# illini-robomaster/irmv_detection

Measured on AMD Instinct MI355X. Metric: end-to-end FPS (preprocess→NMS→PnP) 640×640 YOLOv8n, 1/2/4/8 MI355X, higher is better.
Workload: dtype f16

## Files before the change

include/irmv_hip.h:

```cpp
#ifndef IRMV_HIP_H
#define IRMV_HIP_H

#include <stddef.h>
#include <stdint.h>

#ifdef __cplusplus
extern "C" {
#endif

#define IRMV_OK 0
#define IRMV_ERR_ARG (-1)
#define IRMV_ERR_HIP (-2)
#define IRMV_ERR_MODEL (-3)

#define IRMV_RESIZE_STRETCH 0
#define IRMV_RESIZE_LETTERBOX 1

#define IRMV_ARMOR_SMALL 0
#define IRMV_ARMOR_LARGE 1

#define IRMV_POINTS_AUTO 0
#define IRMV_POINTS_KEYPOINT_HEAD 1
#define IRMV_POINTS_CLASSICAL 2

// ... 119 lines not shown
int irmv_engine_detect(irmv_engine *e, int slot, irmv_det *out, int cap, int *n);
double irmv_engine_last_detect_ms(const irmv_engine *e);

int irmv_engine_rotated_image(irmv_engine *e, int slot, uint8_t *dst_hwc);

int irmv_engine_extract_armors(irmv_engine *e, int slot, const float *xyxy, int n, irmv_det *out);
int irmv_engine_set_extract_params(irmv_engine *e, int binary_threshold, float light_min_ratio, float light_max_ratio,
                                   float light_max_angle, const double center_distances[4]);
int irmv_engine_point_source(const irmv_engine *e);

int irmv_engine_read_input(irmv_engine *e, int slot, float *chw);
int irmv_engine_read_head(irmv_engine *e, int slot, float *head);
int irmv_engine_write_head(irmv_engine *e, int slot, const float *head);
int irmv_engine_run_post(irmv_engine *e, int first_slot, int count);
int irmv_engine_debug_poke_candidate_counts(irmv_engine *e, int value);
int irmv_engine_read_tap(irmv_engine *e, int slot, const char *name, float *nhwc, int shape[3]);
int irmv_engine_read_raw(irmv_engine *e, int slot, irmv_raw_dets *out);
int irmv_engine_num_anchors(const irmv_engine *e);
int irmv_engine_head_channels(const irmv_engine *e);
int irmv_engine_net_dims(const irmv_engine *e, int *width, int *height);

typedef struct irmv_conv_seg {
    char tensor[32];
    int32_t coff, C, shift;
} irmv_conv_seg;

typedef struct irmv_conv_op {
    int32_t op;
    char layer[32];
    int32_t ks, stride, act, out_f32, cin, cout, cout_pad;
// ... 86 lines not shown
```

irmv_detection_amd/capi.py:

```python
from __future__ import annotations

import ctypes as C
import os

from . import _build

OK, ERR_ARG, ERR_HIP, ERR_MODEL = 0, -1, -2, -3
RESIZE_STRETCH, RESIZE_LETTERBOX = 0, 1
ARMOR_SMALL, ARMOR_LARGE = 0, 1
SUBMIT_H2D = 1
SUBMIT_ASYNC_UPLOAD = 2
POINTS_AUTO, POINTS_KEYPOINT_HEAD, POINTS_CLASSICAL = 0, 1, 2
SRC_HWC8, SRC_BAYER_RGGB8, SRC_BAYER_BGGR8, SRC_BAYER_GRBG8, SRC_BAYER_GBRG8 = 0, 1, 2, 3, 4
BAYER_FORMATS = {"RGGB": SRC_BAYER_RGGB8, "BGGR": SRC_BAYER_BGGR8, "GRBG": SRC_BAYER_GRBG8, "GBRG": SRC_BAYER_GBRG8}
NUM_CLASSES = 14
MAX_DET_CAP = 256
CAND_CAP = 8192


class IrmvError(RuntimeError):
    def __init__(self, code: int, msg: str):
        super().__init__(f"irmv_hip error {code}: {msg}")
        self.code = code

# ... 119 lines not shown
    ("irmv_engine_wait_upload", C.c_int, [_P, C.c_int, C.c_int]),
    ("irmv_engine_set_extract_params", C.c_int, [_P, C.c_int, C.c_float, C.c_float, C.c_float, C.POINTER(C.c_double)]),
    ("irmv_engine_point_source", C.c_int, [_P]),
    ("irmv_engine_results", C.c_int, [_P, C.c_int, C.POINTER(Det), C.c_int, C.POINTER(C.c_int)]),
    ("irmv_engine_detect", C.c_int, [_P, C.c_int, C.POINTER(Det), C.c_int, C.POINTER(C.c_int)]),
    ("irmv_engine_last_detect_ms", C.c_double, [_P]),
    ("irmv_engine_rotated_image", C.c_int, [_P, C.c_int, C.POINTER(C.c_uint8)]),
    ("irmv_engine_extract_armors", C.c_int, [_P, C.c_int, C.POINTER(C.c_float), C.c_int, C.POINTER(Det)]),
    ("irmv_engine_light_trace", C.c_int, [_P, C.c_int, C.POINTER(C.c_float), C.c_int, C.POINTER(LightTrace), C.POINTER(Det)]),
    ("irmv_light_limits", C.c_int, [C.POINTER(C.c_int32)]),
    ("irmv_engine_read_input", C.c_int, [_P, C.c_int, C.POINTER(C.c_float)]),
    ("irmv_engine_read_head", C.c_int, [_P, C.c_int, C.POINTER(C.c_float)]),
    ("irmv_engine_write_head", C.c_int, [_P, C.c_int, C.POINTER(C.c_float)]),
    ("irmv_engine_run_post", C.c_int, [_P, C.c_int, C.c_int]),
    ("irmv_engine_debug_poke_candidate_counts", C.c_int, [_P, C.c_int]),
    ("irmv_engine_read_tap", C.c_int, [_P, C.c_int, C.c_char_p, C.POINTER(C.c_float), C.POINTER(C.c_int)]),
    ("irmv_engine_read_raw", C.c_int, [_P, C.c_int, C.POINTER(RawDets)]),
    ("irmv_engine_num_anchors", C.c_int, [_P]),
    ("irmv_engine_head_channels", C.c_int, [_P]),
    ("irmv_engine_net_dims", C.c_int, [_P, C.POINTER(C.c_int), C.POINTER(C.c_int)]),
    ("irmv_engine_conv_ops", C.c_int, [_P, C.POINTER(ConvOp), C.c_int, C.POINTER(C.c_int)]),
    ("irmv_engine_conv_candidates", C.c_int, [_P, C.c_int, C.c_int, C.POINTER(ConvCand), C.c_int, C.POINTER(C.c_int)]),
    ("irmv_engine_run_conv_candidate", C.c_int, [_P, C.c_int, C.c_int, C.c_int, C.c_int, C.c_int, C.c_uint32]),
    ("irmv_engine_read_tensor", C.c_int, [_P, C.c_char_p, C.c_int, C.c_int, C.c_void_p, C.c_size_t]),
    ("irmv_engine_ops", C.c_int, [_P, C.POINTER(GraphOp), C.c_int, C.POINTER(C.c_int)]),
    ("irmv_engine_run_op", C.c_int, [_P, C.c_int, C.c_int, C.c_int, C.c_uint32]),
    ("irmv_sppf_slab", C.c_int, [C.c_int, C.c_int, C.c_int, C.c_int]),
    ("irmv_engine_profile", C.c_int, [_P, C.c_int, C.c_int, C.POINTER(KernelStat), C.c_int, C.POINTER(C.c_int)]),
    ("irmv_pnp_create", C.c_int, [C.c_int, C.POINTER(C.c_double), C.POINTER(C.c_double), C.POINTER(_P)]),
    ("irmv_pnp_destroy", None, [_P]),
# ... 64 lines not shown
```

irmv_detection_amd/csrc/engine.cpp:

```cpp
#include <hip/hip_runtime.h>

#include <algorithm>
#include <chrono>
#include <cmath>
#include <cstdio>
#include <cstring>
#include <fstream>
#include <map>
#include <mutex>
#include <set>
#include <memory>
#include <string>
#include <vector>

#include "../../include/irmv_hip.h"
#include "irmv_common.hpp"
#include "numa.hpp"

using namespace irmv;

static thread_local std::string g_err;
static int fail(int code, const std::string &msg)
{
    g_err = msg;
// ... 133 lines not shown
    bool fused_away = false;
    int group = -1;
    int bneck = -1;
    int kpt3 = -1;
    int tune_fuse[2] = {-1, -1};
};

enum StepKind { STEP_BATCH, STEP_ONE, STEP_MATERIALIZE, STEP_POST };

struct Launch {
    int op = -1, group = -1;
    bool cfg_one = false;
    bool fused = false;
    unsigned scan = 0;
    bool keys_only = false;
    bool once = false;
    std::string name, layer;
    double flops = 0, bytes = 0, launch_bytes = 0;
};

struct GraphKey {
    int first, count;
    StepKind kind;
    bool upload;
    bool operator<(const GraphKey &o) const { return std::tie(first, count, kind, upload) < std::tie(o.first, o.count, o.kind, o.upload); }
};

struct SlotGroup {
    int first = 0, count = 0;
    hipEvent_t h2d = nullptr, out = nullptr;
// ... 3 lines not shown
};

struct irmv_engine {
    irmv_engine_cfg cfg{};
    int nc = 0, nk = 0, A = 0, no = 0;
    int backbone = 0;
    int num_cus = 256;
    int numa_node = -1;
    bool numa_placed = false;
    struct HeadGroup { std::vector<int> members; int family = 0, nt = 1; ConvCfg cfg{}; char name[48] = {0}; };
    std::vector<HeadGroup> head_groups;
    bool post_keys_only = false;
    bool emit_scan = false;
    bool split_scan = true;
    int *cand_counts = nullptr;
    int lvl_hw[3] = {0, 0, 0}, lvl_base[3] = {0, 0, 0};
    size_t frame_bytes = 0;
    size_t src_bytes = 0;
    hipStream_t stream = nullptr;
    hipStream_t extra_streams[7] = {nullptr, nullptr, nullptr, nullptr, nullptr, nullptr, nullptr};
    int num_streams = 1;
    hipStream_t h2d_stream = nullptr;
    std::map<std::pair<int, int>, SlotGroup> groups;
    std::vector<SlotGroup *> slot_owner;
    bool inline_copies = false;
    bool graph_upload = true;
    uint8_t *src_host = nullptr;
    int sync_launch = 0;
    uint8_t *src_host_dev = nullptr;
    int upload_kernel_blocks = 256;
// ... 813 lines not shown
                if (!(fh && fh[0] == '0') && o1.cout == 64 && o1.cin % 32 == 0 && o1.pair && o1.res_t < 0 && o1.cfg.stride == 1 &&
                    o2.cin == 64 && o2.ksteps == 2 && o2.cfg.ks == 1 && o2.cfg.out_f32 && o2.cfg.act == 0 && (o2.cout_pad == 16 || o2.cout_pad == 64))
                    e->ops[i1].fuse_next = i2;
                if (!(fh && fh[0] == '0') && o1.cfg.cin16 && o1.cout_pad == 16 && !o1.pair && o1.res_t < 0 && o1.cfg.stride == 1 && o1.cfg.act == 1 && o2.w_k16)
                    e->ops[i1].fuse_next = i2;
            }
            if (b == 2 && !e->merge_head0) TRY(fuse_kpt3(e, i));
        }

    TRY(dev_alloc(e, (void **)&e->boxes, (size_t)S * e->A * 16));
    TRY(dev_alloc(e, (void **)&e->keys, (size_t)S * e->A * e->nc * 8));
    { const char *sp = getenv("IRMV_SPLIT_SCAN"); e->split_scan = !(sp && sp[0] == '0'); }
    if (e->split_scan) {
        TRY(dev_alloc(e, (void **)&e->cand_counts, (size_t)S * sizeof(int)));
        HIP_TRY(hipMemset(e->cand_counts, 0, (size_t)S * sizeof(int)));
    }
    TRY(dev_alloc(e, (void **)&e->dets_dev, (size_t)S * c.max_det * sizeof(DevDet)));
    TRY(dev_alloc(e, (void **)&e->fout_dev, (size_t)S * sizeof(DevFrameOut)));
    HIP_TRY(hipMemset(e->dets_dev, 0, (size_t)S * c.max_det * sizeof(DevDet)));
    HIP_TRY(hipMemset(e->fout_dev, 0, (size_t)S * sizeof(DevFrameOut)));
    HIP_TRY(hipHostMalloc((void **)&e->dets_host, (size_t)S * c.max_det * sizeof(DevDet), hipHostMallocMapped | hipHostMallocCoherent));
    HIP_TRY(hipHostMalloc((void **)&e->fout_host, (size_t)S * sizeof(DevFrameOut), hipHostMallocMapped | hipHostMallocCoherent));
    HIP_TRY(hipHostGetDevicePointer((void **)&e->dets_host_dev, e->dets_host, 0));
    HIP_TRY(hipHostGetDevicePointer((void **)&e->fout_host_dev, e->fout_host, 0));
    log_range(e, "pinned dets_host", e->dets_host, (size_t)S * c.max_det * sizeof(DevDet));
    log_range(e, "pinned fout_host", e->fout_host, (size_t)S * sizeof(DevFrameOut));
    memset(e->dets_host, 0, (size_t)S * c.max_det * sizeof(DevDet));
    memset(e->fout_host, 0, (size_t)S * sizeof(DevFrameOut));
    if (e->split_scan) {
        Op op; op.kind = OP_SCAN; op.layer = "scan_decode"; snprintf(op.kname, sizeof op.kname, "scan_decode");
        op.bytes = (double)e->A * 64.0; e->ops.push_back(op);
// ... 536 lines not shown
    for (Op &op : e->ops) {
        if (op.fuse_next < 0) continue;
        const bool k16 = op.cfg.cin16 && !op.cfg.lds && !op.cfg_one.lds && !op.cfg.deep && !op.cfg_one.deep && op.cfg.nt == 1 && op.cfg_one.nt == 1 && e->ops[op.fuse_next].w_k16;
        const bool ok = k16 || (op.cfg.lds && op.cfg.nt == 4 && op.cfg_one.lds && op.cfg_one.nt == 4);
        if (!ok) { op.fuse_next = -1; continue; }
        e->ops[op.fuse_next].fused_away = true;
        e->lazy_tensors.insert(e->tensors[op.out_t].name);
        const size_t l = strlen(op.kname), l1 = strlen(op.kname_one);
        snprintf(op.kname + l, sizeof op.kname - l, "+1x1");
        snprintf(op.kname_one + l1, sizeof op.kname_one - l1, "+1x1");
    }
    int fused = 0;
    for (const Op &op : e->ops) fused += is_cls_final_carrier(op);
    const char *ev = getenv("IRMV_EMIT_SCAN");
    e->emit_scan = e->split_scan && fused == 3 && !(ev && ev[0] == '0');
}

static void scan_args_for(const irmv_engine *e, const Op &op, const PostArgs &pa, ConvArgs &a)
{
    a.scan_keys = pa.keys; a.scan_counts = pa.counts; a.scan_thr = pa.logit_thr; a.scan_nc = pa.nc;
    a.scan_key_cap = pa.key_cap;
    a.scan_abase = e->lvl_base[op.level];
}

static bool launch_head_group(const irmv_engine *e, const irmv_engine::HeadGroup &g, int first, const PostArgs *pa, unsigned scan, hipStream_t s)
{
    ConvArgs a[kMultiMax];
    ConvWeights w[kMultiMax];
    const int n = (int)g.members.size();
    for (int k = 0; k < n; k++) {
        const Op &op = e->ops[g.members[k]];
        fill_conv_args(e, op, first, 1, a[k], true);
        if (scan >> k & 1u) scan_args_for(e, op, *pa, a[k]);
        w[k] = conv_weights(op);
    }
    return g.family == 0 ? launch_conv_lds_multi(g.nt, a, w, n, 1, s) : launch_conv_direct_multi(g.cfg, a, n, s);
}
// ... 81 lines not shown
        if (kpt) { g3.push_back(find_op("model.22.cv4." + si + ".1")); g4.push_back(find_op("model.22.cv4." + si + ".2")); }
    }
    try_group(g1, 0, {1, 2}, "head_s0");
    if (g2_fused) try_group(g2, 0, {4}, "head_s1+1x1");
    if (kpt) {
        const size_t before = e->head_groups.size();
        try_group(g3, 1, {1}, "head_kpt1");
        bool k16 = false;
        for (int i : g4) k16 = k16 || i < 0 || e->ops[i].w_k16 != nullptr;
        if (e->head_groups.size() > before && !k16) try_group(g4, 1, {1}, "head_kpt2");
    }
    HIP_TRY(hipStreamSynchronize(e->stream));
    return IRMV_OK;
}

static void build_step_plans(irmv_engine *e)
{
    for (int k = STEP_BATCH; k <= STEP_POST; k++) {
        const bool one = k == STEP_ONE, mat = k == STEP_MATERIALIZE, post = k == STEP_POST, step = !mat && !post;
        auto emits = [&](const Op &op) { return step && e->emit_scan && is_cls_final_carrier(op); };
        for (int i = 0; i < (int)e->ops.size(); i++) {
            const Op &op = e->ops[i];
            if (post && op.kind != OP_NMS && op.kind != OP_LIGHT && op.kind != OP_SCAN) continue;
            if (op.kind == OP_SCAN && e->emit_scan && !post) continue;
            const bool grouped = one && op.kind == OP_CONV && op.group >= 0;
            if (grouped && e->head_groups[op.group].members[0] != i) continue;
            const bool bneck = one && e->bneck64;
            if (op.kind == OP_BNECK ? !bneck : (op.bneck >= 0 && bneck)) continue;
            if (op.kind == OP_KPT3 ? !step : (op.kpt3 >= 0 && step)) continue;
            if (mat ? !(op.fused_away || op.fuse_next >= 0 || ((op.bneck >= 0 || op.kpt3 >= 0) && op.kind == OP_CONV)) : op.fused_away) continue;
// ... 12 lines not shown
                    l.flops += mo.flops + (mo.fuse_next >= 0 ? e->ops[mo.fuse_next].flops : 0.0);
                    l.bytes += mo.bytes;
                }
            } else {
                l.cfg_one = op.kind == OP_CONV && (one || mat) && stream_share(e, e->cfg.num_slots) > 1;
                l.fused = !mat && op.fuse_next >= 0;
                l.scan = emits(op) ? 1u : 0u;
                l.name = l.cfg_one ? op.kname_one : op.kname;
                const Op *nx = l.fused ? &e->ops[op.fuse_next] : nullptr;
                l.flops = op.flops + (nx ? nx->flops : 0.0);
                l.launch_bytes = op.w_bytes + (nx ? nx->w_bytes : 0.0);
                l.bytes = op.bytes + (nx ? nx->out_bytes - op.out_bytes + nx->w_bytes : 0.0) - l.launch_bytes;
            }
            e->plans[k].push_back(l);
        }
    }
}

struct EvRec { hipEvent_t a = nullptr, b = nullptr; };
constexpr int kProfileRepeat = 4;

static void fill_conv_args(const irmv_engine *e, const Op &op, int first, int count, ConvArgs &a, bool fused)
{
    a = ConvArgs{};
    auto seg = [&](const SegRef &s) {
        ConvSeg cs{nullptr, 0, 0, 0};
        if (s.t < 0 || s.C == 0) return cs;
        const Tensor &t = e->tensors[s.t];
        cs.p = static_cast<const half_t *>(t.slot(first)) + s.coff;
        cs.ld = t.C;
// ... 69 lines not shown
}

static PostArgs post_args(const irmv_engine *e, int first)
{
    PostArgs p = e->post;
    p.head_all = e->head_all;
    p.slots_total = e->cfg.num_slots;
    p.first = first;
    p.boxes = e->boxes + (size_t)first * e->A * 4;
    p.keys = e->keys + (size_t)first * e->A * e->nc;
    p.key_cap = e->A * e->nc;
    p.dets = (e->zero_copy_results ? e->dets_host_dev : e->dets_dev) + (size_t)first * e->cfg.max_det;
    p.fout = (e->zero_copy_results ? e->fout_host_dev : e->fout_dev) + first;
    if (p.dbg) p.dbg += (size_t)first * 16;
    p.counts = e->split_scan ? e->cand_counts + first : nullptr;
    return p;
}

static bool launch_c2f32_op(const irmv_engine *e, const Op &op, int first, int count, hipStream_t s)
{
    C2f32Args a{};
    const Tensor &ct = e->tensors[op.res_t];
    const Tensor &ot = e->tensors[op.out_t];
    if (op.sub[0] >= 0) {
        ConvArgs ca;
        fill_conv_args(e, e->ops[op.sub[0]], first, count, ca, false);
        a.s0 = ca.s0; a.s1 = ca.s1; a.cin1 = ca.Cin;
        a.w_cv1 = e->ops[op.sub[0]].w_packed; a.b_cv1 = e->ops[op.sub[0]].bias;
    } else {
        a.cin1 = 32;
// ... 127 lines not shown
            }
            if (!launch_bneck64(op.mode, ks2, op.shortcut, a, count, s)) return fail(IRMV_ERR_ARG, "no fused bottleneck kernel for " + op.layer);
            break;
        }
        case OP_KPT3: {
            const Op &o0 = e->ops[op.sub[0]], &o1 = e->ops[op.sub[1]], &o2 = e->ops[op.sub[2]];
            const Tensor &xt = e->tensors[o0.s0.t], &ht = e->tensors[o2.out_t];
            Kpt3Args a{};
            a.x = static_cast<const half_t *>(xt.slot(first)) + o0.s0.coff; a.x_ld = xt.C;
            a.H = op.Hin; a.W = op.Win;
            a.tiles_x = (op.Win + kKpt3Tile - 1) / kKpt3Tile; a.tiles_y = (op.Hin + kKpt3Tile - 1) / kKpt3Tile;
            a.w1 = o0.w_lds[0]; a.b1 = o0.bias;
            a.w2 = o1.w_packed; a.b2 = o1.bias;
            a.w3 = o2.w_k16; a.b3 = o2.bias;
            a.out = static_cast<float *>(ht.slot(first)) + o2.out_coff; a.out_ld = ht.C;
            if (!launch_kpt3(a, op.cin, count, s)) return fail(IRMV_ERR_ARG, "no fused keypoint-branch kernel for " + op.layer);
            break;
        }
        case OP_DW: case OP_SHUF: case OP_CONV0: case OP_POOL: launch_graph_op(e, op, first, count, s); break;
        case OP_CONV: {
            const unsigned scan = rep == n - 1 ? l.scan : 0u;
            if (l.group >= 0) {
                if (!launch_head_group(e, e->head_groups[l.group], first, &pa, scan, s)) return fail(IRMV_ERR_ARG, "grouped launch refused: " + l.name);
                break;
            }
            ConvArgs a;
            fill_conv_args(e, op, first, count, a, l.fused);
            if (scan) scan_args_for(e, op, pa, a);
            if (!run_conv(op, l.cfg_one ? op.cfg_one : op.cfg, a, count, s)) return fail(IRMV_ERR_ARG, std::string("no conv kernel for ") + op.kname + " (" + op.layer + ")");
            break;
        }
        case OP_SCAN: launch_scan_decode(pa, count, s); break;
        case OP_NMS: { PostArgs pn = pa; pn.keys_only = l.keys_only ? 1 : 0; launch_nms_pnp(pn, count, s); break; }
        case OP_LIGHT: launch_light_extract(light_args(e, first), e->cfg.max_det, count, s); break;
        }
        HIP_TRY(hipGetLastError());
        if (ev) {
            HIP_TRY(hipEventRecord(r.b, s));
            ev->push_back(r);
        }
    }
    return IRMV_OK;
}
// ... 95 lines not shown
        if (up != st) HIP_TRY(hipStreamWaitEvent(up, o->out, 0));
    }
    if (g->in_flight && g->compute != st) HIP_TRY(hipStreamWaitEvent(st, g->out, 0));
    if (flags & IRMV_SUBMIT_H2D) {
        if (async_up) {
            if (g->in_flight) HIP_TRY(hipStreamWaitEvent(up, g->out, 0));
            TRY(copy_in(e, f, c, up));
            HIP_TRY(hipEventRecord(g->h2d, up));
            HIP_TRY(hipStreamWaitEvent(st, g->h2d, 0));
        } else if (!graph_up) {
            TRY(upload_sync(e, f, c, st));
        }
    }
    if (eager) TRY(enqueue_step(e, kind, f, c, st, 1, nullptr));
    else HIP_TRY(hipGraphLaunch(ge, st));
    TRY(copy_out(e, f, c, st));
    HIP_TRY(hipEventRecord(g->out, st));
    g->in_flight = true;
    g->async_up = async_up;
    g->compute = st;
    return IRMV_OK;
}

extern "C" int irmv_engine_submit(irmv_engine *e, int first, int count, uint32_t flags)
{
    TRY(check_range(e, first, count));
    HIP_TRY(hipSetDevice(e->cfg.device));
    int share = count > 1 ? stream_share(e, count) : count;
    int si = count == 1 ? first % e->num_streams : 0;
    const int full_share = stream_share(e, e->cfg.num_slots);
// ... 7 lines not shown
}

extern "C" int irmv_engine_wait(irmv_engine *e);

extern "C" int irmv_engine_debug_poke_candidate_counts(irmv_engine *e, int value)
{
    if (!e) return fail(IRMV_ERR_ARG, "engine is null");
    if (!e->cand_counts) return fail(IRMV_ERR_ARG, "this engine keeps no candidate counters");
    TRY(irmv_engine_wait(e));
    HIP_TRY(hipSetDevice(e->cfg.device));
    std::vector<int> v((size_t)e->cfg.num_slots, value);
    HIP_TRY(hipMemcpy(e->cand_counts, v.data(), v.size() * sizeof(int), hipMemcpyHostToDevice));
    return IRMV_OK;
}

extern "C" int irmv_engine_run_post(irmv_engine *e, int first, int count)
{
    TRY(check_range(e, first, count));
    HIP_TRY(hipSetDevice(e->cfg.device));
    TRY(irmv_engine_wait(e));
    hipGraphExec_t ge;
    TRY(get_graph(e, STEP_POST, first, count, false, &ge));
    HIP_TRY(hipGraphLaunch(ge, e->stream));
    TRY(copy_out(e, first, count));
    HIP_TRY(hipStreamSynchronize(e->stream));
    return IRMV_OK;
}

extern "C" int irmv_engine_wait(irmv_engine *e)
{
    if (!e) return fail(IRMV_ERR_ARG, "engine is null");
    HIP_TRY(hipSetDevice(e->cfg.device));
    HIP_TRY(hipStreamSynchronize(e->h2d_stream));
    HIP_TRY(hipStreamSynchronize(e->stream));
    for (int i = 1; i < e->num_streams; i++) HIP_TRY(hipStreamSynchronize(e->extra_streams[i - 1]));
// ... 200 lines not shown
        std::vector<uint16_t> h(t.slot_elems);
        HIP_TRY(hipMemcpy(h.data(), t.slot(slot), t.slot_elems * 2, hipMemcpyDeviceToHost));
        const float unscale = t.name == "input" ? 1.0f : kActUnscale;
        for (size_t i = 0; i < t.slot_elems; i++) out[i] = half_bits_to_float(h[i]) * unscale;
    }
    return IRMV_OK;
}

static int materialize_fused(irmv_engine *e, int slot)
{
    if (e->lazy_tensors.empty()) return IRMV_OK;
    HIP_TRY(hipSetDevice(e->cfg.device));
    TRY(irmv_engine_wait(e));
    TRY(enqueue_step(e, STEP_MATERIALIZE, slot, 1, e->stream, 1, nullptr));
    HIP_TRY(hipStreamSynchronize(e->stream));
    return IRMV_OK;
}

extern "C" int irmv_engine_read_input(irmv_engine *e, int slot, float *chw)
{
    TRY(check_range(e, slot, 1));
    TRY(materialize_fused(e, slot));
    std::vector<float> v;
    TRY(read_tensor_f32(e, e->tensors[e->tensor_idx.at("input")], slot, v));
    const size_t n = (size_t)e->cfg.net_size * e->cfg.net_height;
    for (size_t p = 0; p < n; p++)
        for (int c = 0; c < 3; c++) chw[c * n + p] = v[p * 4 + c];
    return IRMV_OK;
}

extern "C" int irmv_engine_read_head(irmv_engine *e, int slot, float *head)
{
    TRY(check_range(e, slot, 1));
    for (int l = 0; l < 3; l++) {
        std::vector<float> v;
        TRY(read_tensor_f32(e, e->tensors[e->head_t[l]], slot, v));
        for (int p = 0; p < e->lvl_hw[l]; p++) {
            float *o = head + (size_t)(e->lvl_base[l] + p) * e->no;
            const float *r = v.data() + (size_t)p * kHeadRec;
            memcpy(o, r, 64 * 4);
            memcpy(o + 64, r + kClsOff, (size_t)e->nc * 4);
            if (e->nk) memcpy(o + 64 + e->nc, r + kKptOff, (size_t)e->nk * 4);
        }
    }
    return IRMV_OK;
}

extern "C" int irmv_engine_write_head(irmv_engine *e, int slot, const float *head)
{
    TRY(check_range(e, slot, 1));
    HIP_TRY(hipSetDevice(e->cfg.device));
    TRY(irmv_engine_wait(e));
    for (int l = 0; l < 3; l++) {
        std::vector<float> v((size_t)e->lvl_hw[l] * kHeadRec, 0.f);
        for (int p = 0; p < e->lvl_hw[l]; p++) {
            const float *o = head + (size_t)(e->lvl_base[l] + p) * e->no;
            float *r = v.data() + (size_t)p * kHeadRec;
            memcpy(r, o, 64 * 4);
            memcpy(r + kClsOff, o + 64, (size_t)e->nc * 4);
            if (e->nk) memcpy(r + kKptOff, o + 64 + e->nc, (size_t)e->nk * 4);
        }
        HIP_TRY(hipMemcpy(e->tensors[e->head_t[l]].slot(slot), v.data(), v.size() * 4, hipMemcpyHostToDevice));
    }
    return IRMV_OK;
}

extern "C" int irmv_engine_read_tap(irmv_engine *e, int slot, const char *name, float *nhwc, int shape[3])
{
    TRY(check_range(e, slot, 1));
    if (!name || !shape) return fail(IRMV_ERR_ARG, "name/shape is null");
    auto it = e->tensor_idx.find(name);
    if (it == e->tensor_idx.end()) return fail(IRMV_ERR_ARG, std::string("no tensor named ") + name);
    const Tensor &t = e->tensors[it->second];
    shape[0] = t.H; shape[1] = t.W; shape[2] = t.C;
    if (!nhwc) return IRMV_OK;
    if (e->lazy_tensors.count(t.name)) TRY(materialize_fused(e, slot));
    std::vector<float> v;
    TRY(read_tensor_f32(e, t, slot, v));
    memcpy(nhwc, v.data(), v.size() * 4);
    return IRMV_OK;
}

extern "C" int irmv_engine_read_tensor(irmv_engine *e, const char *name, int first, int count, void *dst, size_t bytes)
{
    TRY(check_range(e, first, count));
    if (!name) return fail(IRMV_ERR_ARG, "name is null");
    auto it = e->tensor_idx.find(name);
    if (it == e->tensor_idx.end()) return fail(IRMV_ERR_ARG, std::string("no tensor named ") + name);
    const Tensor &t = e->tensors[it->second];
    const size_t need = t.slot_elems * t.esize() * count;
    if (!dst || bytes != need) return fail(IRMV_ERR_ARG, "read_tensor: buffer size does not match the slot range");
    TRY(irmv_engine_wait(e));
    HIP_TRY(hipMemcpy(dst, t.slot(first), need, hipMemcpyDeviceToHost));
    return IRMV_OK;
}

static int conv_op_at(const irmv_engine *e, int op)
{
    if (!e) return fail(IRMV_ERR_ARG, "engine is null");
    if (op < 0 || op >= (int)e->ops.size() || e->ops[op].kind != OP_CONV) return fail(IRMV_ERR_ARG, "not a conv op");
    return IRMV_OK;
}

extern "C" int irmv_engine_conv_ops(irmv_engine *e, irmv_conv_op *ops, int cap, int *n)
{
    if (!e || !n) return fail(IRMV_ERR_ARG, "engine / n is null");
    auto name = [](char *dst, size_t cap_, const std::string &s) { snprintf(dst, cap_, "%s", s.c_str()); };
// ... 224 lines not shown
        if (out->det_anchors) out->det_anchors[i] = d[i].anchor;
        if (out->det_kpts) memcpy(out->det_kpts + 8 * i, d[i].kpts_net, 32);
    }
    return IRMV_OK;
}

extern "C" int irmv_engine_profile(irmv_engine *e, int first, int count, irmv_kernel_stat *stats, int cap, int *n)
{
    TRY(check_range(e, first, count));
    if (!n) return fail(IRMV_ERR_ARG, "n is null");
    HIP_TRY(hipSetDevice(e->cfg.device));
    TRY(irmv_engine_wait(e));
    const StepKind kind = count == 1 ? STEP_ONE : STEP_BATCH;
    std::vector<EvRec> ev;
    TRY(enqueue_step(e, kind, first, count, e->stream, kProfileRepeat, &ev));
    TRY(copy_out(e, first, count));
    HIP_TRY(hipStreamSynchronize(e->stream));
    for (size_t i = 0; i < ev.size(); i++) {
        float ms = 0.f;
        HIP_TRY(hipEventElapsedTime(&ms, ev[i].a, ev[i].b));
        (void)hipEventDestroy(ev[i].a);
        (void)hipEventDestroy(ev[i].b);
        const Launch &l = e->plans[kind][i];
        if ((int)i < cap && stats) {
            irmv_kernel_stat &st = stats[i];
            memset(&st, 0, sizeof st);
            snprintf(st.name, sizeof st.name, "%s", l.name.c_str());
            snprintf(st.layer, sizeof st.layer, "%s", l.layer.c_str());
            st.flops = l.flops * count;
            st.bytes = l.bytes * count + l.launch_bytes;
// ... 78 lines not shown
```

irmv_detection_amd/csrc/irmv_common.hpp:

```cpp
#pragma once

#include <hip/hip_runtime.h>

#include <cstdint>
#include <cstdlib>

namespace irmv {

typedef _Float16 half_t;
typedef _Float16 half8 __attribute__((ext_vector_type(8)));
typedef _Float16 half4 __attribute__((ext_vector_type(4)));
typedef float f32x4 __attribute__((ext_vector_type(4)));

constexpr float kActScale = 1.44269504088896341f;
constexpr float kActUnscale = 0.693147180559945309f;
typedef unsigned int u32x4_t __attribute__((ext_vector_type(4)));
__device__ __forceinline__ float silu_rcp(float y) { return __builtin_amdgcn_rcpf(1.0f + __builtin_amdgcn_exp2f(-y)); }
__device__ __forceinline__ unsigned int silu_pack2(float y0, float y1)
{
    const float r0 = silu_rcp(y0), r1 = silu_rcp(y1);
    unsigned int o;
    asm("v_fma_mixlo_f16 %0, %1, %2, 0" : "=v"(o) : "v"(y0), "v"(r0));
    asm("v_fma_mixhi_f16 %0, %1, %2, 0" : "+v"(o) : "v"(y1), "v"(r1));
    return o;
// ... 180 lines not shown
bool launch_bneck64(int mode, int ks2, bool shortcut, const BneckArgs &a, int batch, hipStream_t s);

constexpr int kKpt3Tile = 10;
struct Kpt3Args {
    const half_t *x;
    int x_ld;
    int H, W, tiles_x, tiles_y;
    const half_t *w1;
    const float *b1;
    const half_t *w2;
    const float *b2;
    const half_t *w3;
    const float *b3;
    float *out;
    int out_ld;
};
bool kpt3_eligible(int cin);
bool launch_kpt3(const Kpt3Args &a, int cin, int batch, hipStream_t s);

struct ConvArgs {
    ConvSeg s0, s1;
    int Hin, Win;
    int Hout, Wout;
    int M;
    int Cin;
    const half_t *w;
    const float *bias;
    void *out;
    int out_ld;
    const half_t *res;
    int res_ld;
    int cout_pad;
    int ksteps;
    int pair;
    const half_t *w2;
    const float *bias2;
    float *out2;
    int out2_ld, n2;
    unsigned long long *scan_keys;
    int *scan_counts;
    float scan_thr;
    int scan_nc, scan_abase, scan_key_cap;
};

constexpr int kMultiMax = 6;
struct LdsMember {
    ConvArgs a;
    const half_t *wl;
    int tiles_x, tiles_y, twc_log2, patch_bytes, batch, tile2d;
    int gx, gy;
};
struct LdsMultiArgs {
    int n;
    int start[kMultiMax + 1];
    LdsMember m[kMultiMax];
};
struct DirectMultiArgs {
// ... 55 lines not shown
    unsigned long long *keys;
    int key_cap;
    DevDet *dets;
    DevFrameOut *fout;
    int net_w, net_h, A, nc, nk;
    float logit_thr, iou_thr;
    int max_det, pre_nms_cap;
    float scale_x, scale_y, off_x, off_y;
    int armor_size;
    const PnpConst *pnp;
    long long *dbg;
    int keys_only;
    int prefilter;
    int classwalk;
    int *counts;
};
void launch_nms_pnp(const PostArgs &a, int batch, hipStream_t s);
constexpr int kScanBlocks = 16;
constexpr size_t kScanLdsMax = 159 * 1024;
void launch_scan_decode(const PostArgs &a, int batch, hipStream_t s);
constexpr int kLightLdsPoints = 256;
constexpr int kLightLdsImage = 40 * 1024;
constexpr int kLightMaxContours = 1024;
constexpr int kLightPointsCap = 4096;

struct LightTraceRec {
    float corners[8];
    float top[2], bottom[2], center[2];
    double length;
    int32_t measured, ok, hull_edges, in_lds;
// ... 40 lines not shown
```

irmv_detection_amd/csrc/k_conv.hip:

```cpp
#include "irmv_common.hpp"

#include <algorithm>
#include <cstdio>
#include <cstring>
#include <iterator>
#include <mutex>
#include <type_traits>

namespace irmv {

template <int MT, int NT>
struct PrefetchDepth { static constexpr int value = (MT * NT >= 8) ? 2 : ((MT * NT >= 4) ? 3 : 4); };
template <int MT, int NT>
struct DeepPrefetchDepth { static constexpr int value = (MT + NT <= 2) ? 12 : ((MT + NT <= 3) ? 10 : 6); };


template <int KS, int STRIDE, int MT, int NT, bool CIN16, int ACT, bool OUT_F32, bool CT = false, bool DEEP = false>
__device__ __forceinline__ void conv_mfma_body(const ConvArgs &a, int wg_x, int wg_y, int grid_x, int grid_y)
{
    constexpr int PAD = KS / 2;
    constexpr int PF = DEEP ? DeepPrefetchDepth<MT, NT>::value : PrefetchDepth<MT, NT>::value;
    static_assert(!CT || (KS == 3 && !CIN16), "chunk-major order is the 3x3 LDS family's");
    const int lane = threadIdx.x & 63, wave = threadIdx.x >> 6;
    const int g = lane >> 4, r = lane & 15;
// ... 818 lines not shown
            for (int mt = 0; mt < MT; mt++) {
                const size_t m = (size_t)im * HWo + mloc[mt];
                if constexpr (NT % 2 == 0) {
#pragma unroll
                    for (int u = 0; u < NT / 2; u++) rv8[mt][u] = *reinterpret_cast<const half8 *>(a.res + m * a.res_ld + (nt0 / 2 + u) * 32 + g * 8);
                } else {
                    const int c0 = a.pair ? ((nt0 >> 1) * 32 + g * 8 + (nt0 & 1) * 4) : (nt0 * 16 + g * 4);
                    rv4[mt] = *reinterpret_cast<const half4 *>(a.res + m * a.res_ld + c0);
                }
            }
        }
#pragma unroll
        for (int mt = 0; mt < MT; mt++) {
            if (N2 > 0 || mv[mt]) {
                const size_t m = (size_t)im * HWo + mloc[mt];
                if constexpr (NT % 2 == 0) {
                    half8 ov[NT / 2];
#pragma unroll
                    for (int u = 0; u < NT / 2; u++) {
                        const int c0 = (nt0 / 2 + u) * 32 + g * 8;
                        float vals[8];
#pragma unroll
                        for (int i = 0; i < 4; i++) {
                            vals[i] = accx[mt][2 * u][i];
                            vals[4 + i] = accx[mt][2 * u + 1][i];
                        }
                        if (a.res) {
#pragma unroll
                            for (int i = 0; i < 8; i++) ov[u][i] = silu_add_res(vals[i], (float)rv8[mt][u][i]);
                        } else {
                            ov[u] = silu_pack8(vals[0], vals[1], vals[2], vals[3], vals[4], vals[5], vals[6], vals[7]);
                        }
                        if constexpr (N2 == 0) *reinterpret_cast<half8 *>(static_cast<half_t *>(a.out) + m * a.out_ld + c0) = ov[u];
                    }
                    if constexpr (N2 > 0) {
                        mfma_operand_fence(ov[0], ov[1]);
#pragma unroll
                        for (int t2 = 0; t2 < N2; t2++) {
                            f32x4 c2 = (f32x4){0.f, 0.f, 0.f, 0.f};
                            c2 = __builtin_amdgcn_mfma_f32_16x16x32_f16(W2[t2][0], ov[0], c2, 0, 0, 0);
                            c2 = __builtin_amdgcn_mfma_f32_16x16x32_f16(W2[t2][1], ov[1], c2, 0, 0, 0);
                            const int co = t2 * 16 + g * 4;
                            const f32x4 b2 = *reinterpret_cast<const f32x4 *>(s_bias2 + co);
                            const f32x4 v2 = (f32x4){c2[0] * kActUnscale + b2[0], c2[1] * kActUnscale + b2[1], c2[2] * kActUnscale + b2[2], c2[3] * kActUnscale + b2[3]};
                            if (mv[mt]) *reinterpret_cast<f32x4 *>(a.out2 + m * a.out2_ld + co) = v2;
                            if (a.scan_keys) {
                                bool hit = false;
#pragma unroll
                                for (int i = 0; i < 4; i++) hit = hit || (mv[mt] && co + i < a.scan_nc && v2[i] > a.scan_thr);
                                if (hit) {
                                    const int an = a.scan_abase + mloc[mt];
#pragma unroll
                                    for (int i = 0; i < 4; i++) {
                                        if (co + i < a.scan_nc && v2[i] > a.scan_thr) {
                                            const int idx = atomicAdd(&a.scan_counts[im], 1);
                                            const unsigned int u = __float_as_uint(v2[i]);
                                            const unsigned int ord = (u & 0x80000000u) ? ~u : (u | 0x80000000u);
                                            if (idx >= 0 && idx < a.scan_key_cap)
                                                a.scan_keys[(size_t)im * a.scan_key_cap + idx] =
                                                    ((unsigned long long)ord << 32) | (unsigned long long)(0xffffffffu - (unsigned int)(an * a.scan_nc + co + i));
                                        }
                                    }
                                }
                            }
                        }
                    }
// ... 611 lines not shown
```

irmv_detection_amd/csrc/k_kpt.hip:

```cpp
#include "irmv_common.hpp"

namespace irmv {

namespace {
constexpr int KT = kKpt3Tile;
constexpr int K1W = KT + 4, K1N = K1W * K1W;
constexpr int K2W = KT + 2, K2N = K2W * K2W;
constexpr int KPL = K1N * 64;
constexpr int KQS = 32;
constexpr int KNT = 192;
constexpr int KNP = (K1N * 8 + KNT - 1) / KNT;
static_assert(K2N == 9 * 16, "the halo region is nine MFMA tiles");
typedef unsigned int u32x4 __attribute__((ext_vector_type(4)));
}

template <int STEPS>
__global__ __launch_bounds__(KNT) __attribute__((amdgpu_waves_per_eu(3))) void kpt3_kernel(Kpt3Args a, int batch, int ipw, int xcd)
{
    extern __shared__ __attribute__((aligned(16))) uint8_t smem[];
    uint8_t *s_in = smem;
    uint8_t *s_t = smem + 2 * KPL;
    half8 *s_w2 = reinterpret_cast<half8 *>(smem + 2 * KPL + K2N * KQS);
    const int tid = threadIdx.x, lane = tid & 63, wave = tid >> 6;
    const int g = lane >> 4, r = lane & 15;
// ... 63 lines not shown
    int toff2[5];
#pragma unroll
    for (int ks = 0; ks < 5; ks++) {
        const int tap = 2 * ks + tap_lo, tc = tap < 9 ? tap : 0, kh = tc / 3, kw = tc - kh * 3;
        toff2[ks] = ((bly + kh) * K2W + blx + kw) * KQS + (g & 1) * 16;
    }
    half8 Bf[2][3];
    auto frag = [&](int kk, half8 (&B)[3]) {
        const int c = kk / 9, tap = kk - c * 9, kh = tap / 3, kw = tap - kh * 3;
        const int off = (kh * K1W + kw) * 64 + c * KPL;
#pragma unroll
        for (int i = 0; i < 3; i++) B[i] = *reinterpret_cast<const half8 *>(s_in + (kh == 1 ? baseO : baseE) + off + i * 256);
    };

    for (int im = 0; im < nimg; im++) {
        f32x4 acc[3] = {b1, b1, b1};
#pragma unroll
        for (int s = 0; s < STEPS; s++) {
            write_slab();
            __syncthreads();
            frag(0, Bf[0]);
#pragma unroll
            for (int kk = 0; kk < 18; kk++) {
                const int k = s * 18 + kk;
                if (kk + 1 < 18) frag(kk + 1, Bf[(kk + 1) & 1]);
                __builtin_amdgcn_sched_barrier(0);
#pragma unroll
                for (int i = 0; i < 3; i++) acc[i] = __builtin_amdgcn_mfma_f32_16x16x32_f16(A[kk % 6], Bf[kk & 1][i], acc[i], 0, 0, 0);
                __builtin_amdgcn_sched_barrier(0);
                if (kk == 12) issue_slab();
// ... 22 lines not shown
            const bool valid = ly < KT && lx < KT;
            f32x4 c1 = b2;
            half8 B2[5];
#pragma unroll
            for (int ks = 0; ks < 5; ks++) {
                const u32x4 q = *reinterpret_cast<const u32x4 *>(s_t + toff2[ks] + i * 4 * KQS);
                B2[ks] = __builtin_bit_cast(half8, 2 * ks + tap_lo < 9 ? q : (u32x4){0u, 0u, 0u, 0u});
            }
#pragma unroll
            for (int ks = 0; ks < 5; ks++) c1 = __builtin_amdgcn_mfma_f32_16x16x32_f16(A2[ks], B2[ks], c1, 0, 0, 0);
            half4 o = silu_pack4(c1[0], c1[1], c1[2], c1[3]);
            mfma_operand_fence(o);
            const f32x4 c2 = __builtin_amdgcn_mfma_f32_16x16x16f16(w3f, o, (f32x4){0.f, 0.f, 0.f, 0.f}, 0, 0, 0);
            const f32x4 v2 = (f32x4){c2[0] * kActUnscale + b3[0], c2[1] * kActUnscale + b3[1], c2[2] * kActUnscale + b3[2], c2[3] * kActUnscale + b3[3]};
            const int gy = oy0 + ly, gx = ox0 + lx;
            if (valid && gy < H && gx < W) *reinterpret_cast<f32x4 *>(a.out + ((size_t)((img0 + im) * H + gy) * W + gx) * a.out_ld + g * 4) = v2;
        }
    }
}

bool kpt3_eligible(int cin) { return cin == 64 || cin == 128 || cin == 256; }

bool launch_kpt3(const Kpt3Args &a, int cin, int batch, hipStream_t s)
{
    const int tiles = a.tiles_x * a.tiles_y;
    int ipw = 1;
    while (ipw < 8 && (long long)tiles * batch >= 2048LL * ipw) ipw *= 2;
    const dim3 grid(tiles * ((batch + ipw - 1) / ipw)), block(KNT);
    constexpr size_t lds = (size_t)2 * KPL + (size_t)K2N * KQS + 4608;
    static_assert(lds <= 40 * 1024, "four workgroups per CU");
    const int xcd = xcd_image_order();
// ... 10 lines not shown
```

irmv_detection_amd/csrc/k_post.hip:

```cpp
#include "irmv_common.hpp"
#include "pnp_device.hpp"

#include <mutex>

namespace irmv {

__device__ __forceinline__ float irmv_expf(float x)
{
    x = x < -87.0f ? -87.0f : x;
    x = x > 88.0f ? 88.0f : x;
    const float n = rintf(x * 1.44269504088896341f);
    float r = fmaf(n, -0.693145751953125f, x);
    r = fmaf(n, -1.42860682030941723212e-6f, r);
    float p = 1.0f / 720.0f;
    p = fmaf(p, r, 1.0f / 120.0f);
    p = fmaf(p, r, 1.0f / 24.0f);
    p = fmaf(p, r, 1.0f / 6.0f);
    p = fmaf(p, r, 0.5f);
    p = fmaf(p, r, 1.0f);
    p = fmaf(p, r, 1.0f);
    return __int_as_float(__float_as_int(p) + ((int)n << 23));
}

__device__ __forceinline__ uint32_t orderable(float f)
// ... 321 lines not shown
        unsigned long long k_mine[KPL];
#pragma unroll
        for (int k = 0; k < KPL; k++) {
            const int i = tid + k * 1024;
            k_mine[k] = gk[i < a.key_cap ? i : a.key_cap - 1];
        }
        int n = a.counts[b];
        n = n < 0 ? 0 : (n > a.key_cap ? a.key_cap : n);
        if (n <= kCandCap) {
#pragma unroll
            for (int k = 0; k < KPL; k++)
                if (tid + k * 1024 < n) skeys[tid + k * 1024] = k_mine[k];
        }
        __syncthreads();
        if (tid == 0) { s_ncand = n; a.counts[b] = 0; }
    } else {
    {
        constexpr int U = 8;
        int lbase = 0;
#pragma unroll 1
        for (int l = 0; l < 3; l++) {
            const int lhw = (a.net_w / (8 << l)) * (a.net_h / (8 << l));
            const float *lrec = a.head_all + ((size_t)lbase * a.slots_total + (size_t)(a.first + b) * lhw) * kHeadRec;
            const int quads = lhw * 4;
            for (int q0 = 0; q0 < quads; q0 += 1024 * U) {
                f32x4 cl[U];
#pragma unroll
                for (int u = 0; u < U; u++) {
                    const int t = q0 + u * 1024 + tid;
                    const int rin = t < quads ? (t >> 2) : 0;
// ... 799 lines not shown
```

irmv_detection_amd/engine.py:

```python
from __future__ import annotations

import ctypes as C
import enum
import os
from dataclasses import dataclass, field
from typing import List, Optional, Sequence, Tuple

import numpy as np

from . import capi
from .capi import IrmvError


class ArmorClass(enum.IntEnum):
    B1 = 0; B2 = 1; B3 = 2; B4 = 3; B5 = 4; BO = 5; BS = 6
    R1 = 7; R2 = 8; R3 = 9; R4 = 10; R5 = 11; RO = 12; RS = 13
    UNKNOWN = 14


class ArmorSize(enum.IntEnum):
    SMALL = 0; LARGE = 1; UNKNOWN = 2


@dataclass
# ... 271 lines not shown
        md = self.max_det
        boxes = np.zeros((md, 4), np.float32); scores = np.zeros(md, np.float32)
        classes = np.zeros(md, np.int32); anchors = np.zeros(md, np.int32); kpts = np.zeros((md, 8), np.float32)
        raw = capi.RawDets(0, 0, boxes.ctypes.data_as(C.POINTER(C.c_float)), scores.ctypes.data_as(C.POINTER(C.c_float)),
                           classes.ctypes.data_as(C.POINTER(C.c_int32)), anchors.ctypes.data_as(C.POINTER(C.c_int32)),
                           kpts.ctypes.data_as(C.POINTER(C.c_float)))
        capi.check(self._L.irmv_engine_read_raw(self._h, slot, C.byref(raw)))
        n = raw.num_dets
        return dict(num_dets=n, n_candidates=raw.n_candidates, boxes=boxes[:n], scores=scores[:n],
                    classes=classes[:n], anchors=anchors[:n], kpts=kpts[:n],
                    boxes_padded=boxes, scores_padded=scores)

    def debug_poke_candidate_counts(self, value: int) -> None:
        capi.check(self._L.irmv_engine_debug_poke_candidate_counts(self._h, int(value)))

    def profile(self, first_slot: int = 0, count: Optional[int] = None) -> List[dict]:
        count = self.num_slots - first_slot if count is None else count
        stats = (capi.KernelStat * 256)()
        n = C.c_int(0)
        capi.check(self._L.irmv_engine_profile(self._h, first_slot, count, stats, 256, C.byref(n)))
        return [dict(name=stats[i].name.decode(), layer=stats[i].layer.decode(), flops=stats[i].flops,
                     bytes=stats[i].bytes, ms=stats[i].ms) for i in range(min(n.value, 256))]

    def _detect_raw(self, slot):
        slot = self.slot if slot is None else slot
        n = C.c_int(0)
        capi.check(self._L.irmv_engine_detect(self._h, slot, self._dets, self.max_det, C.byref(n)))
        return [self._dets[i] for i in range(n.value)]

    @staticmethod
# ... 49 lines not shown
```

Measured before the change: 61170.

## Gate box and keypoint head stores on per-anchor candidate bitmask

The class-score scan kernel now sets a per-frame bitmask of anchors whose class logits pass the threshold. The box-branch conv and the keypoint kernel check this mask and write head outputs only for candidate anchors. The launch plan is reordered so box convs run after the last class scan. The goal is to cut head output write traffic, at the cost of extra mask reads, atomics, a mask clear in the post kernel, and lazy re-materialisation of the dense head when debug readers need it.

```diff
diff --git a/include/irmv_hip.h b/include/irmv_hip.h
--- a/include/irmv_hip.h
+++ b/include/irmv_hip.h
@@ -157,6 +157,7 @@
 int irmv_engine_write_head(irmv_engine *e, int slot, const float *head);
 int irmv_engine_run_post(irmv_engine *e, int first_slot, int count);
 int irmv_engine_debug_poke_candidate_counts(irmv_engine *e, int value);
+int irmv_engine_debug_read_cand_bits(irmv_engine *e, int slot, uint32_t *words, int cap, int *n, int *sparse);
 int irmv_engine_read_tap(irmv_engine *e, int slot, const char *name, float *nhwc, int shape[3]);
 int irmv_engine_read_raw(irmv_engine *e, int slot, irmv_raw_dets *out);
 int irmv_engine_num_anchors(const irmv_engine *e);
diff --git a/irmv_detection_amd/capi.py b/irmv_detection_amd/capi.py
--- a/irmv_detection_amd/capi.py
+++ b/irmv_detection_amd/capi.py
@@ -157,6 +157,7 @@
     ("irmv_engine_write_head", C.c_int, [_P, C.c_int, C.POINTER(C.c_float)]),
     ("irmv_engine_run_post", C.c_int, [_P, C.c_int, C.c_int]),
     ("irmv_engine_debug_poke_candidate_counts", C.c_int, [_P, C.c_int]),
+    ("irmv_engine_debug_read_cand_bits", C.c_int, [_P, C.c_int, C.POINTER(C.c_uint32), C.c_int, C.POINTER(C.c_int), C.POINTER(C.c_int)]),
     ("irmv_engine_read_tap", C.c_int, [_P, C.c_int, C.c_char_p, C.POINTER(C.c_float), C.POINTER(C.c_int)]),
     ("irmv_engine_read_raw", C.c_int, [_P, C.c_int, C.POINTER(RawDets)]),
     ("irmv_engine_num_anchors", C.c_int, [_P]),
diff --git a/irmv_detection_amd/csrc/engine.cpp b/irmv_detection_amd/csrc/engine.cpp
--- a/irmv_detection_amd/csrc/engine.cpp
+++ b/irmv_detection_amd/csrc/engine.cpp
@@ -171,6 +171,7 @@
     bool fused = false;
     unsigned scan = 0;
     bool keys_only = false;
+    bool sparse = false;
     bool once = false;
     std::string name, layer;
     double flops = 0, bytes = 0, launch_bytes = 0;
@@ -204,6 +205,10 @@
     bool emit_scan = false;
     bool split_scan = true;
     int *cand_counts = nullptr;
+    bool sparse_head = false;
+    unsigned int *cand_bits = nullptr;
+    int cand_words = 0;
+    std::vector<char> head_stale;
     int lvl_hw[3] = {0, 0, 0}, lvl_base[3] = {0, 0, 0};
     size_t frame_bytes = 0;
     size_t src_bytes = 0;
@@ -1047,7 +1052,11 @@
     if (e->split_scan) {
         TRY(dev_alloc(e, (void **)&e->cand_counts, (size_t)S * sizeof(int)));
         HIP_TRY(hipMemset(e->cand_counts, 0, (size_t)S * sizeof(int)));
-    }
+        e->cand_words = (e->A + 31) / 32;
+        TRY(dev_alloc(e, (void **)&e->cand_bits, (size_t)S * e->cand_words * sizeof(unsigned int)));
+        HIP_TRY(hipMemset(e->cand_bits, 0, (size_t)S * e->cand_words * sizeof(unsigned int)));
+    }
+    e->head_stale.assign((size_t)S, 0);
     TRY(dev_alloc(e, (void **)&e->dets_dev, (size_t)S * c.max_det * sizeof(DevDet)));
     TRY(dev_alloc(e, (void **)&e->fout_dev, (size_t)S * sizeof(DevFrameOut)));
     HIP_TRY(hipMemset(e->dets_dev, 0, (size_t)S * c.max_det * sizeof(DevDet)));
@@ -1614,6 +1623,8 @@
     for (const Op &op : e->ops) fused += is_cls_final_carrier(op);
     const char *ev = getenv("IRMV_EMIT_SCAN");
     e->emit_scan = e->split_scan && fused == 3 && !(ev && ev[0] == '0');
+    const char *sh = getenv("IRMV_SPARSE_HEAD");
+    e->sparse_head = e->emit_scan && e->cand_bits && !(sh && sh[0] == '0');
 }
 
 static void scan_args_for(const irmv_engine *e, const Op &op, const PostArgs &pa, ConvArgs &a)
@@ -1621,6 +1632,7 @@
     a.scan_keys = pa.keys; a.scan_counts = pa.counts; a.scan_thr = pa.logit_thr; a.scan_nc = pa.nc;
     a.scan_key_cap = pa.key_cap;
     a.scan_abase = e->lvl_base[op.level];
+    a.cand_bits = pa.cand_bits; a.cand_words = pa.cand_words;
 }
 
 static bool launch_head_group(const irmv_engine *e, const irmv_engine::HeadGroup &g, int first, const PostArgs *pa, unsigned scan, hipStream_t s)
@@ -1732,6 +1744,36 @@
     return IRMV_OK;
 }
 
+static bool is_box_final_carrier(const Op &op) { return op.fuse_next >= 0 && op.level >= 0 && op.layer.rfind("model.22.cv2.", 0) == 0; }
+
+static void sparse_head_plan(const irmv_engine *e, std::vector<Launch> &plan)
+{
+    int last_cls = -1;
+    bool lvl_cls[3] = {false, false, false};
+    for (size_t i = 0; i < plan.size(); i++)
+        if (plan[i].scan && plan[i].group < 0) { last_cls = (int)i; lvl_cls[e->ops[plan[i].op].level] = true; }
+    std::vector<Launch> out, moved;
+    for (size_t i = 0; i < plan.size(); i++) {
+        Launch &l = plan[i];
+        const Op &op = e->ops[l.op];
+        if (l.scan) {
+            if (l.group < 0) l.bytes -= e->ops[op.fuse_next].out_bytes;
+            else for (size_t m = 0; m < e->head_groups[l.group].members.size(); m++)
+                if (l.scan >> m & 1u) l.bytes -= e->ops[e->ops[e->head_groups[l.group].members[m]].fuse_next].out_bytes;
+        }
+        const bool cls_first = op.level >= 0 && op.level < 3 && lvl_cls[op.level];
+        const bool box = l.group < 0 && l.fused && op.kind == OP_CONV && is_box_final_carrier(op) && cls_first;
+        const bool kpt = op.kind == OP_KPT3 && cls_first && (int)i > last_cls;
+        if (box || kpt) {
+            l.sparse = true;
+            l.bytes -= box ? e->ops[op.fuse_next].out_bytes : op.out_bytes;
+        }
+        if (box && (int)i < last_cls) moved.push_back(l); else out.push_back(l);
+        if ((int)i == last_cls) { out.insert(out.end(), moved.begin(), moved.end()); moved.clear(); }
+    }
+    plan.swap(out);
+}
+
 static void build_step_plans(irmv_engine *e)
 {
     for (int k = STEP_BATCH; k <= STEP_POST; k++) {
@@ -1774,6 +1816,7 @@
             }
             e->plans[k].push_back(l);
         }
+        if (step && e->sparse_head) sparse_head_plan(e, e->plans[k]);
     }
 }
 
@@ -1873,6 +1916,8 @@
     p.fout = (e->zero_copy_results ? e->fout_host_dev : e->fout_dev) + first;
     if (p.dbg) p.dbg += (size_t)first * 16;
     p.counts = e->split_scan ? e->cand_counts + first : nullptr;
+    p.cand_bits = e->sparse_head ? e->cand_bits + (size_t)first * e->cand_words : nullptr;
+    p.cand_words = e->cand_words;
     return p;
 }
 
@@ -2030,19 +2075,23 @@
             a.w2 = o1.w_packed; a.b2 = o1.bias;
             a.w3 = o2.w_k16; a.b3 = o2.bias;
             a.out = static_cast<float *>(ht.slot(first)) + o2.out_coff; a.out_ld = ht.C;
+            if (l.sparse) { a.cand_bits = pa.cand_bits; a.cand_words = pa.cand_words; a.abase = e->lvl_base[op.level]; }
             if (!launch_kpt3(a, op.cin, count, s)) return fail(IRMV_ERR_ARG, "no fused keypoint-branch kernel for " + op.layer);
             break;
         }
         case OP_DW: case OP_SHUF: case OP_CONV0: case OP_POOL: launch_graph_op(e, op, first, count, s); break;
         case OP_CONV: {
-            const unsigned scan = rep == n - 1 ? l.scan : 0u;
+            unsigned scan = rep == n - 1 ? l.scan : 0u;
+            PostArgs pr = pa;
+            if (!scan && l.scan && e->sparse_head) { scan = l.scan; pr.logit_thr = INFINITY; }
             if (l.group >= 0) {
-                if (!launch_head_group(e, e->head_groups[l.group], first, &pa, scan, s)) return fail(IRMV_ERR_ARG, "grouped launch refused: " + l.name);
+                if (!launch_head_group(e, e->head_groups[l.group], first, &pr, scan, s)) return fail(IRMV_ERR_ARG, "grouped launch refused: " + l.name);
                 break;
             }
             ConvArgs a;
             fill_conv_args(e, op, first, count, a, l.fused);
-            if (scan) scan_args_for(e, op, pa, a);
+            if (scan) scan_args_for(e, op, pr, a);
+            if (l.sparse) { a.cand_bits = pa.cand_bits; a.cand_words = pa.cand_words; a.scan_abase = e->lvl_base[op.level]; }
             if (!run_conv(op, l.cfg_one ? op.cfg_one : op.cfg, a, count, s)) return fail(IRMV_ERR_ARG, std::string("no conv kernel for ") + op.kname + " (" + op.layer + ")");
             break;
         }
@@ -2168,6 +2217,7 @@
     }
     if (eager) TRY(enqueue_step(e, kind, f, c, st, 1, nullptr));
     else HIP_TRY(hipGraphLaunch(ge, st));
+    if (e->sparse_head) std::fill(e->head_stale.begin() + f, e->head_stale.begin() + f + c, 1);
     TRY(copy_out(e, f, c, st));
     HIP_TRY(hipEventRecord(g->out, st));
     g->in_flight = true;
@@ -2205,11 +2255,28 @@
     return IRMV_OK;
 }
 
+extern "C" int irmv_engine_debug_read_cand_bits(irmv_engine *e, int slot, uint32_t *words, int cap, int *n, int *sparse)
+{
+    TRY(check_range(e, slot, 1));
+    if (!n || !sparse) return fail(IRMV_ERR_ARG, "n / sparse is null");
+    *sparse = e->sparse_head ? 1 : 0;
+    *n = e->sparse_head ? e->cand_words : 0;
+    if (!words || *n == 0) return IRMV_OK;
+    if (cap < *n) return fail(IRMV_ERR_ARG, "read_cand_bits: buffer too small");
+    TRY(irmv_engine_wait(e));
+    HIP_TRY(hipSetDevice(e->cfg.device));
+    HIP_TRY(hipMemcpy(words, e->cand_bits + (size_t)slot * e->cand_words, (size_t)e->cand_words * sizeof(unsigned int), hipMemcpyDeviceToHost));
+    return IRMV_OK;
+}
+
+static int ensure_dense_head(irmv_engine *e, int slot);
+
 extern "C" int irmv_engine_run_post(irmv_engine *e, int first, int count)
 {
     TRY(check_range(e, first, count));
     HIP_TRY(hipSetDevice(e->cfg.device));
     TRY(irmv_engine_wait(e));
+    for (int s = first; s < first + count; s++) TRY(ensure_dense_head(e, s));
     hipGraphExec_t ge;
     TRY(get_graph(e, STEP_POST, first, count, false, &ge));
     HIP_TRY(hipGraphLaunch(ge, e->stream));
@@ -2440,6 +2507,14 @@
     TRY(irmv_engine_wait(e));
     TRY(enqueue_step(e, STEP_MATERIALIZE, slot, 1, e->stream, 1, nullptr));
     HIP_TRY(hipStreamSynchronize(e->stream));
+    e->head_stale[slot] = 0;
+    return IRMV_OK;
+}
+
+static int ensure_dense_head(irmv_engine *e, int slot)
+{
+    if (!e->head_stale[slot]) return IRMV_OK;
+    TRY(materialize_fused(e, slot));
     return IRMV_OK;
 }
 
@@ -2458,6 +2533,7 @@
 extern "C" int irmv_engine_read_head(irmv_engine *e, int slot, float *head)
 {
     TRY(check_range(e, slot, 1));
+    TRY(ensure_dense_head(e, slot));
     for (int l = 0; l < 3; l++) {
         std::vector<float> v;
         TRY(read_tensor_f32(e, e->tensors[e->head_t[l]], slot, v));
@@ -2488,6 +2564,7 @@
         }
         HIP_TRY(hipMemcpy(e->tensors[e->head_t[l]].slot(slot), v.data(), v.size() * 4, hipMemcpyHostToDevice));
     }
+    e->head_stale[slot] = 0;
     return IRMV_OK;
 }
 
@@ -2501,6 +2578,7 @@
     shape[0] = t.H; shape[1] = t.W; shape[2] = t.C;
     if (!nhwc) return IRMV_OK;
     if (e->lazy_tensors.count(t.name)) TRY(materialize_fused(e, slot));
+    for (int l = 0; l < 3; l++) if (it->second == e->head_t[l]) TRY(ensure_dense_head(e, slot));
     std::vector<float> v;
     TRY(read_tensor_f32(e, t, slot, v));
     memcpy(nhwc, v.data(), v.size() * 4);
@@ -2517,6 +2595,8 @@
     const size_t need = t.slot_elems * t.esize() * count;
     if (!dst || bytes != need) return fail(IRMV_ERR_ARG, "read_tensor: buffer size does not match the slot range");
     TRY(irmv_engine_wait(e));
+    for (int l = 0; l < 3; l++)
+        if (it->second == e->head_t[l]) for (int s = first; s < first + count; s++) TRY(ensure_dense_head(e, s));
     HIP_TRY(hipMemcpy(dst, t.slot(first), need, hipMemcpyDeviceToHost));
     return IRMV_OK;
 }
@@ -2771,6 +2851,7 @@
     const StepKind kind = count == 1 ? STEP_ONE : STEP_BATCH;
     std::vector<EvRec> ev;
     TRY(enqueue_step(e, kind, first, count, e->stream, kProfileRepeat, &ev));
+    if (e->sparse_head) std::fill(e->head_stale.begin() + first, e->head_stale.begin() + first + count, 1);
     TRY(copy_out(e, first, count));
     HIP_TRY(hipStreamSynchronize(e->stream));
     for (size_t i = 0; i < ev.size(); i++) {
diff --git a/irmv_detection_amd/csrc/irmv_common.hpp b/irmv_detection_amd/csrc/irmv_common.hpp
--- a/irmv_detection_amd/csrc/irmv_common.hpp
+++ b/irmv_detection_amd/csrc/irmv_common.hpp
@@ -218,6 +218,8 @@
     const float *b3;
     float *out;
     int out_ld;
+    const unsigned int *cand_bits;
+    int cand_words, abase;
 };
 bool kpt3_eligible(int cin);
 bool launch_kpt3(const Kpt3Args &a, int cin, int batch, hipStream_t s);
@@ -245,6 +247,8 @@
     int *scan_counts;
     float scan_thr;
     int scan_nc, scan_abase, scan_key_cap;
+    unsigned int *cand_bits;
+    int cand_words;
 };
 
 constexpr int kMultiMax = 6;
@@ -330,6 +334,8 @@
     int prefilter;
     int classwalk;
     int *counts;
+    unsigned int *cand_bits;
+    int cand_words;
 };
 void launch_nms_pnp(const PostArgs &a, int batch, hipStream_t s);
 constexpr int kScanBlocks = 16;
diff --git a/irmv_detection_amd/csrc/k_conv.hip b/irmv_detection_amd/csrc/k_conv.hip
--- a/irmv_detection_amd/csrc/k_conv.hip
+++ b/irmv_detection_amd/csrc/k_conv.hip
@@ -856,6 +856,14 @@
         for (int mt = 0; mt < MT; mt++) {
             if (N2 > 0 || mv[mt]) {
                 const size_t m = (size_t)im * HWo + mloc[mt];
+                bool st2 = mv[mt];
+                if constexpr (N2 > 0) {
+                    const bool gate = a.cand_bits != nullptr && a.scan_keys == nullptr;
+                    const int an = a.scan_abase + mloc[mt];
+                    const unsigned int *cb = gate ? a.cand_bits : reinterpret_cast<const unsigned int *>(a.bias2);
+                    const unsigned int cw = cb[gate ? (unsigned int)(im * a.cand_words + (an >> 5)) : 0u];
+                    st2 = mv[mt] && (a.cand_bits == nullptr || (gate && ((cw >> (an & 31)) & 1u)));
+                }
                 if constexpr (NT % 2 == 0) {
                     half8 ov[NT / 2];
 #pragma unroll
@@ -885,13 +893,14 @@
                             const int co = t2 * 16 + g * 4;
                             const f32x4 b2 = *reinterpret_cast<const f32x4 *>(s_bias2 + co);
                             const f32x4 v2 = (f32x4){c2[0] * kActUnscale + b2[0], c2[1] * kActUnscale + b2[1], c2[2] * kActUnscale + b2[2], c2[3] * kActUnscale + b2[3]};
-                            if (mv[mt]) *reinterpret_cast<f32x4 *>(a.out2 + m * a.out2_ld + co) = v2;
+                            if (st2) *reinterpret_cast<f32x4 *>(a.out2 + m * a.out2_ld + co) = v2;
                             if (a.scan_keys) {
                                 bool hit = false;
 #pragma unroll
                                 for (int i = 0; i < 4; i++) hit = hit || (mv[mt] && co + i < a.scan_nc && v2[i] > a.scan_thr);
                                 if (hit) {
                                     const int an = a.scan_abase + mloc[mt];
+                                    if (a.cand_bits) atomicOr(&a.cand_bits[(size_t)im * a.cand_words + (an >> 5)], 1u << (an & 31));
 #pragma unroll
                                     for (int i = 0; i < 4; i++) {
                                         if (co + i < a.scan_nc && v2[i] > a.scan_thr) {
diff --git a/irmv_detection_amd/csrc/k_kpt.hip b/irmv_detection_amd/csrc/k_kpt.hip
--- a/irmv_detection_amd/csrc/k_kpt.hip
+++ b/irmv_detection_amd/csrc/k_kpt.hip
@@ -101,6 +101,15 @@
     };
 
     for (int im = 0; im < nimg; im++) {
+        unsigned int cw[3];
+#pragma unroll
+        for (int i = 0; i < 3; i++) {
+            const int gy = oy0 + bly, gx = ox0 + i * 4 + blx;
+            const int an = a.abase + ((gy < H && gx < W) ? gy * W + gx : 0);
+            const unsigned int *cb = a.cand_bits ? a.cand_bits : reinterpret_cast<const unsigned int *>(a.b3);
+            const unsigned int w = cb[a.cand_bits ? (unsigned int)((img0 + im) * a.cand_words + (an >> 5)) : 0u];
+            cw[i] = a.cand_bits ? (w >> (an & 31)) & 1u : 1u;
+        }
         f32x4 acc[3] = {b1, b1, b1};
 #pragma unroll
         for (int s = 0; s < STEPS; s++) {
@@ -153,7 +162,7 @@
             const f32x4 c2 = __builtin_amdgcn_mfma_f32_16x16x16f16(w3f, o, (f32x4){0.f, 0.f, 0.f, 0.f}, 0, 0, 0);
             const f32x4 v2 = (f32x4){c2[0] * kActUnscale + b3[0], c2[1] * kActUnscale + b3[1], c2[2] * kActUnscale + b3[2], c2[3] * kActUnscale + b3[3]};
             const int gy = oy0 + ly, gx = ox0 + lx;
-            if (valid && gy < H && gx < W) *reinterpret_cast<f32x4 *>(a.out + ((size_t)((img0 + im) * H + gy) * W + gx) * a.out_ld + g * 4) = v2;
+            if (valid && gy < H && gx < W && cw[i]) *reinterpret_cast<f32x4 *>(a.out + ((size_t)((img0 + im) * H + gy) * W + gx) * a.out_ld + g * 4) = v2;
         }
     }
 }
diff --git a/irmv_detection_amd/csrc/k_post.hip b/irmv_detection_amd/csrc/k_post.hip
--- a/irmv_detection_amd/csrc/k_post.hip
+++ b/irmv_detection_amd/csrc/k_post.hip
@@ -359,6 +359,8 @@
         }
         __syncthreads();
         if (tid == 0) { s_ncand = n; a.counts[b] = 0; }
+        if (a.cand_bits)
+            for (int i = tid; i < a.cand_words; i += blockDim.x) a.cand_bits[(size_t)b * a.cand_words + i] = 0u;
     } else {
     {
         constexpr int U = 8;
diff --git a/irmv_detection_amd/engine.py b/irmv_detection_amd/engine.py
--- a/irmv_detection_amd/engine.py
+++ b/irmv_detection_amd/engine.py
@@ -309,6 +309,15 @@
     def debug_poke_candidate_counts(self, value: int) -> None:
         capi.check(self._L.irmv_engine_debug_poke_candidate_counts(self._h, int(value)))
 
+    def debug_cand_bits(self, slot: int = 0):
+        n, sparse = C.c_int(0), C.c_int(0)
+        capi.check(self._L.irmv_engine_debug_read_cand_bits(self._h, slot, None, 0, C.byref(n), C.byref(sparse)))
+        words = np.zeros(n.value, np.uint32)
+        if n.value:
+            capi.check(self._L.irmv_engine_debug_read_cand_bits(self._h, slot, words.ctypes.data_as(C.POINTER(C.c_uint32)), n.value,
+                                                                 C.byref(n), C.byref(sparse)))
+        return bool(sparse.value), words
+
     def profile(self, first_slot: int = 0, count: Optional[int] = None) -> List[dict]:
         count = self.num_slots - first_slot if count is None else count
         stats = (capi.KernelStat * 256)()
```

Result: faster. 62080, median of 6 (+1.5%).
